# eric-ai-lab/Aerial-Vision-and-Dialog-Navigation

Measured on NVIDIA B200. Metric: HAA-Transformer train episodes/s, higher is better.
Workload: dtype bf16

## Files before the change

### aerial-vision-and-dialog-navigation_b200/_lib.py

```python
from __future__ import annotations

import ctypes as C
import os

import torch

_HERE = os.path.dirname(os.path.abspath(__file__))
LIB_PATH = os.path.join(_HERE, "csrc", "libavdn.so")

_lib = None

c_void_p, c_int, c_i64, c_f32, c_f64 = C.c_void_p, C.c_int, C.c_int64, C.c_float, C.c_double


class ConvItem(C.Structure):
    _fields_ = [("w", C.c_void_p), ("wf", C.c_void_p), ("wd", C.c_void_p), ("dwf", C.c_void_p), ("grad", C.c_void_p),
                ("Cout", C.c_int32), ("Cin", C.c_int32), ("k", C.c_int32), ("stride", C.c_int32),
                ("Cout_p", C.c_int32), ("Cin_p", C.c_int32), ("pairs", C.c_int32), ("pad_", C.c_int32)]


class TileDesc(C.Structure):
    _fields_ = [("tile8", C.c_void_p), ("H", C.c_int32), ("W", C.c_int32)]


_SIGNATURES = {
    "avdn_pack_tile": [c_void_p, c_void_p, c_int, c_int, c_int, c_void_p, c_void_p],
    "avdn_resize_area_width": [c_void_p, c_int, c_int, c_int, c_void_p, c_void_p, c_void_p, c_void_p, c_void_p],
    "avdn_raster_attention": [c_void_p, c_int, c_int, c_void_p, c_int, c_int, c_int, c_void_p, c_void_p],
    "avdn_gps_to_pixels": [c_void_p, c_void_p, c_int, c_void_p, c_void_p],
    "avdn_homography_from_corners": [c_void_p, c_int, c_void_p, c_void_p],
    "avdn_render_views": [c_void_p, c_int, c_void_p, c_void_p, c_int, c_void_p, c_void_p,
                          c_void_p, c_void_p, c_void_p, c_void_p],
    "avdn_gemm_plan": [c_void_p, c_void_p, C.c_size_t],
    "avdn_gemm_run": [c_void_p, c_void_p],
    "avdn_conv0_fwd": [c_void_p, c_void_p, c_void_p, c_int, c_int, c_int, c_void_p, c_void_p],
    "avdn_conv0_fwd_eval": [c_void_p, c_void_p, c_void_p, c_void_p, c_f32, c_void_p, c_int, c_int, c_int, c_void_p],
    "avdn_conv0_wgrad": [c_void_p, c_void_p, c_void_p, c_int, c_int, c_int, c_void_p],
    "avdn_conv0_fwd_stats": [c_void_p, c_void_p, c_int, c_int, c_int, c_void_p, c_void_p, c_void_p, c_void_p],
    "avdn_conv0_fwd_apply": [c_void_p, c_void_p, c_void_p, c_void_p, c_f32, c_void_p, c_void_p, c_int, c_int, c_int,
                             c_void_p],
    "avdn_conv0_set_tensor_path": [c_int],
    "avdn_conv3x3_thin_fwd": [c_void_p, c_void_p, c_void_p, c_int, c_int, c_int, c_int, c_int, c_void_p, c_void_p],
    "avdn_conv3x3_thin_supported": [c_int, c_int, c_int, c_int],
    "avdn_conv3x3_thin_dgrad": [c_void_p, c_void_p, c_void_p, c_int, c_int, c_int, c_int, c_int, c_void_p],
    "avdn_conv3x3_thin_wgrad": [c_void_p, c_void_p, c_void_p, c_int, c_int, c_int, c_int, c_int, c_void_p],
    "avdn_conv0_bwd": [c_void_p] * 8 + [c_f32, c_int, c_int, c_int] + [c_void_p] * 7 + [c_void_p],
    "avdn_bn_stats": [c_void_p, c_i64, c_int, c_int, c_void_p, c_void_p, c_void_p, c_void_p, c_f32, c_f32,
                      c_void_p, c_void_p, c_void_p, c_void_p, c_void_p, c_void_p],
    "avdn_bn_finalize": [c_void_p, c_i64, c_int, c_int, c_void_p, c_void_p, c_void_p, c_void_p, c_f32, c_f32,
                         c_void_p, c_void_p, c_void_p, c_void_p, c_void_p],
    "avdn_bn_eval_coeffs": [c_int, c_int, c_void_p, c_void_p, c_void_p, c_void_p, c_f32, c_void_p, c_void_p,
                            c_void_p],
    "avdn_bn_set_order": [c_int],
    "avdn_bn_apply": [c_void_p, c_void_p, c_void_p, c_void_p, c_void_p, c_i64, c_int, c_f32, c_void_p],
    "avdn_bn_backward": [c_void_p, c_void_p, c_void_p, c_void_p, c_void_p, c_void_p, c_i64, c_int, c_int, c_f32,
                         c_void_p, c_void_p, c_void_p, c_void_p, c_void_p],
    "avdn_bn_backward_apply": [c_void_p, c_void_p, c_void_p, c_void_p, c_void_p, c_void_p, c_i64, c_int, c_int, c_f32,
                               c_void_p, c_void_p, c_void_p, c_void_p, c_void_p, c_void_p],
    "avdn_pack_conv_weight": [c_void_p, c_int, c_int, c_int, c_int, c_int, c_void_p, c_void_p, c_void_p],
    "avdn_unpack_conv_wgrad": [c_void_p, c_int, c_int, c_int, c_int, c_void_p, c_void_p],
    "avdn_unpack_conv_wgrad_pairs": [c_void_p, c_int, c_int, c_int, c_int, c_int, c_int, c_void_p, c_void_p],
    "avdn_pack_conv_weights": [c_void_p, c_int, c_void_p],
    "avdn_unpack_conv_wgrads": [c_void_p, c_int, c_int, c_void_p],
    "avdn_cast_f32_bf16": [c_void_p, c_void_p, c_i64, c_void_p],
    "avdn_nhwc_to_nchw_f32": [c_void_p, c_void_p, c_int, c_int, c_int, c_void_p],
    "avdn_nchw_f32_to_nhwc": [c_void_p, c_void_p, c_int, c_int, c_int, c_void_p],
    "avdn_frame_attn_fwd": [c_void_p] * 6 + [c_int, c_int] + [c_void_p] * 4 + [c_void_p],
    "avdn_frame_attn_bwd": [c_void_p] * 5 + [c_int, c_int] + [c_void_p] * 9 + [c_void_p],
# ... 138 lines not shown
```

### aerial-vision-and-dialog-navigation_b200/csrc/common.cu

```cuda
#include "common.cuh"

#include <stdlib.h>

namespace avdn {

static thread_local char g_err[512] = "ok";

char* err_buf() { return g_err; }

int set_err(int code, const char* fmt, ...) {
  va_list ap;
  va_start(ap, fmt);
  vsnprintf(g_err, sizeof(g_err), fmt, ap);
  va_end(ap);
  return code;
}

int check_launch(const char* what) {
  cudaError_t e = cudaGetLastError();
  if (e != cudaSuccess)
    return set_err(AVDN_ERR_LAUNCH, "%s: %s", what, cudaGetErrorString(e));
  return AVDN_OK;
}

// ... 1 lines not shown
  static int n = 0;
  if (n == 0) {
    int dev = 0;
    if (cudaGetDevice(&dev) != cudaSuccess) return 148;
    cudaDeviceProp p;
    if (cudaGetDeviceProperties(&p, dev) != cudaSuccess) return 148;
    n = p.multiProcessorCount;
  }
  return n;
}

bool pdl_enabled() {
  static const bool on = [] {
    const char* e = getenv("AVDN_PDL");
    return e && e[0] == '1';
  }();
  return on;
}

}

extern "C" const char* avdn_last_error_string(void) { return avdn::err_buf(); }

extern "C" int avdn_abi_version(void) { return 11; }

extern "C" int avdn_device_supported(void) {
  int n = 0;
  if (cudaGetDeviceCount(&n) != cudaSuccess || n == 0) {
    cudaGetLastError();
    return 0;
  }
  cudaDeviceProp p;
  if (cudaGetDeviceProperties(&p, 0) != cudaSuccess) return 0;
  return p.major == 10 ? 1 : 0;
}
```

### aerial-vision-and-dialog-navigation_b200/csrc/conv3_halo.cu

```cuda
#include "common.cuh"
#include "tcgen05.cuh"
#include "conv3_halo.cuh"

namespace {

using namespace avdn_tc;

constexpr int TW = 8, TH = 16;
constexpr int THREADS = 128;

template <int CIN, int COUT, int XBUFS>
struct Cfg {
  static constexpr int ROW = CIN * 2;
  static constexpr int ATOM = 8 * ROW;
  static constexpr int XBOX = (TH + 2) * ATOM;
  static constexpr int XBUF = 3 * XBOX;
  static constexpr int WTAP = COUT * ROW;
  static constexpr int WBYTES = 9 * WTAP;
  static constexpr int OUT_ROW = COUT * 2;
  static constexpr int OUT_BYTES = 128 * OUT_ROW;
  static constexpr int NCH = OUT_ROW / 16;
  static constexpr uint32_t LAYOUT = (CIN == 64) ? 2u : 4u;
  static constexpr int SMEM = XBUFS * XBUF + WBYTES + 2 * OUT_BYTES + 1024;
  static constexpr uint32_t IDESC = (1u << 4) | (1u << 7) | (1u << 10) | ((uint32_t)(COUT >> 3) << 17) | ((uint32_t)(128 >> 4) << 24);
  static constexpr uint32_t TMEM_COLS = COUT < 32 ? 32 : COUT;
// ... 270 lines not shown
    }
  }
  __syncwarp();
  if (n_my > 0) {
    mbar_wait(bar_done, 0);
    tcgen05_fence_after();
    const int co = (int)warp * 16 + (int)lane;
#pragma unroll
    for (int h = 0; h < 9; ++h) {
      uint32_t v[32];
      tmem_ld32(tmem + ((warp * 32u) << 16) + 32 * h, v);
      if (lane < 16) {
        const int kh = h / 3, kw = h % 3;
#pragma unroll
        for (int ci = 0; ci < 32; ++ci) atomicAdd(p.dw + ((co * CIN + ci) * 3 + kh) * 3 + kw, __uint_as_float(v[ci]));
      }
    }
  }
  tcgen05_fence_before();
  __syncthreads();
  if (warp == 0) asm volatile("tcgen05.dealloc.cta_group::1.sync.aligned.b32 %0, %1;" ::"r"(tmem), "r"(512u) : "memory");
}

}

namespace avdn {

static bool tile_ok(int H, int W) { return H % TH == 0 && W % TW == 0 && H >= TH && W >= TW; }

bool conv3_halo_supported(int H, int W, int Cin, int Cout) { return Cin == 32 && Cout == 64 && tile_ok(H, W); }
bool conv3_halo_dgrad_supported(int H, int W, int Cin, int Cout) { return Cin == 32 && Cout == 64 && tile_ok(H, W); }

int conv3_halo_fwd(const void* x, const void* wf, void* z, int N, int H, int W, int Cin, int Cout, double* stats,
                   cudaStream_t s) {
  if (!conv3_halo_supported(H, W, Cin, Cout))
    return set_err(AVDN_ERR_UNSUPPORTED, "conv3_halo: shape %dx%d, %d -> %d channels not covered", H, W, Cin, Cout);
  return stats ? launch<32, 64, false, true, 1>(x, wf, z, N, H, W, stats, s)
               : launch<32, 64, false, false, 1>(x, wf, z, N, H, W, nullptr, s);
}

int conv3_halo_dgrad(const void* dz, const void* wd, void* dx, int N, int H, int W, int Cin, int Cout, cudaStream_t s) {
  if (!conv3_halo_dgrad_supported(H, W, Cin, Cout))
    return set_err(AVDN_ERR_UNSUPPORTED, "conv3_halo dgrad: shape %dx%d, %d -> %d channels not covered", H, W, Cin, Cout);
  return launch<64, 32, true, false, 1>(dz, wd, dx, N, H, W, nullptr, s);
}

int conv3_halo_wgrad(const void* dz, const void* x, float* dw, int N, int H, int W, int Cin, int Cout, cudaStream_t s) {
  if (!conv3_halo_supported(H, W, Cin, Cout))
    return set_err(AVDN_ERR_UNSUPPORTED, "conv3_halo wgrad: shape %dx%d, %d -> %d channels not covered", H, W, Cin, Cout);
  WgParams p;
  const int64_t dx[4] = {Cin, W, H, N}, sx[4] = {1, Cin, (int64_t)W * Cin, (int64_t)H * W * Cin};
  const int32_t bx[4] = {Cin, TW, TH + 2, 1};
  const int64_t dd[4] = {Cout, W, H, N}, sd[4] = {1, Cout, (int64_t)W * Cout, (int64_t)H * W * Cout};
  const int32_t bd[4] = {Cout, TW, TH, 1};
  int r = encode_tensor_map_4d(x, 2, dx, sx, bx, &p.tmX);
  if (!r) r = encode_tensor_map_4d(dz, 2, dd, sd, bd, &p.tmDz);
  if (r) return r;
  p.tiles_x = W / TW;
  p.tiles_y = H / TH;
  const long long nt = (long long)N * p.tiles_x * p.tiles_y;
  if (nt >= (1ll << 31)) return set_err(AVDN_ERR_UNSUPPORTED, "conv3_halo wgrad: too many tiles");
  p.n_tiles = (int32_t)nt;
  p.dw = dw;
  const int smem = WG_STAGES * (3 * (TH + 2) * 8 * 64 + 128 * 128) + 1024;
  static bool attr = false;
  if (!attr) {
    if (cudaFuncSetAttribute(conv3_halo_wgrad_kernel, cudaFuncAttributeMaxDynamicSharedMemorySize, smem) != cudaSuccess)
// ... 8 lines not shown
}

extern "C" int avdn_conv3x3_thin_wgrad(const void* dz, const void* x_nhwc, float* dw, int N, int H, int W, int Cin,
                                       int Cout, avdn_stream_t stream) {
  AVDN_REQUIRE(dz && x_nhwc && dw && N > 0, "avdn_conv3x3_thin_wgrad: bad argument");
  return avdn::conv3_halo_wgrad(dz, x_nhwc, dw, N, H, W, Cin, Cout, avdn::to_cuda(stream));
}

extern "C" int avdn_conv3x3_thin_fwd(const void* x_nhwc, const void* w_f, void* z, int N, int H, int W, int Cin,
                                     int Cout, double* stats, avdn_stream_t stream) {
  AVDN_REQUIRE(x_nhwc && w_f && z && N > 0, "avdn_conv3x3_thin_fwd: bad argument");
  return avdn::conv3_halo_fwd(x_nhwc, w_f, z, N, H, W, Cin, Cout, stats, avdn::to_cuda(stream));
}

extern "C" int avdn_conv3x3_thin_dgrad(const void* dz, const void* w_d, void* dx, int N, int H, int W, int Cin,
                                       int Cout, avdn_stream_t stream) {
  AVDN_REQUIRE(dz && w_d && dx && N > 0, "avdn_conv3x3_thin_dgrad: bad argument");
  return avdn::conv3_halo_dgrad(dz, w_d, dx, N, H, W, Cin, Cout, avdn::to_cuda(stream));
}

extern "C" int avdn_conv3x3_thin_supported(int H, int W, int Cin, int Cout) {
  return avdn::conv3_halo_supported(H, W, Cin, Cout) ? 1 : 0;
}
```

### aerial-vision-and-dialog-navigation_b200/csrc/conv3_halo.cuh

```cuda
#pragma once
#include "common.cuh"

#include <cuda.h>

namespace avdn {

int encode_tensor_map_4d(const void* ptr, int elem_bytes, const int64_t* dim, const int64_t* stride,
                         const int32_t* boxdim, CUtensorMap* out);

bool conv3_halo_supported(int H, int W, int Cin, int Cout);
int conv3_halo_fwd(const void* x, const void* wf, void* z, int N, int H, int W, int Cin, int Cout, double* stats,
                   cudaStream_t s);
bool conv3_halo_dgrad_supported(int H, int W, int Cin, int Cout);
int conv3_halo_dgrad(const void* dz, const void* wd, void* dx, int N, int H, int W, int Cin, int Cout, cudaStream_t s);

int conv3_halo_wgrad(const void* dz, const void* x, float* dw, int N, int H, int W, int Cin, int Cout, cudaStream_t s);

}
```

### aerial-vision-and-dialog-navigation_b200/models/dark_net.py

```python
from __future__ import annotations

import os

import torch
import torch.nn as nn

from .. import _lib
from .. import gemm as G

LEAKY_SLOPE = 0.01
FUSE_BNB = os.environ.get("AVDN_FUSE_BNB", "0") == "1"
CONV0_RECOMPUTE = os.environ.get("AVDN_CONV0_RECOMPUTE", "1") != "0"
CONV_HALO = os.environ.get("AVDN_CONV_HALO", "1") != "0"
BN_EPS = 1e-5
BN_MOMENTUM = 0.1


def parse_model_config(path):
    defs = []
    with open(path, "r") as f:
        for raw in f.read().split("\n"):
            line = raw.strip()
            if not line or line.startswith("#"):
                continue
            if line.startswith("["):
                d = {"type": line[1:-1].rstrip()}
                if d["type"] == "convolutional":
                    d["batch_normalize"] = 0
                defs.append(d)
            else:
                k, v = line.split("=")
                defs[-1][k.rstrip()] = v.strip()
    return defs


def _pad64(c):
# ... 46 lines not shown
        defs = net.module_defs
        out_of = {}
        cur = dict(C=3, Cp=4, H=H, W=W, layer=None)
        shapes = {}
        max_elems = 0
        for i, d in enumerate(defs):
            if d["type"] == "convolutional":
                conv = net.module_list[i][0]
                if int(d["batch_normalize"]) != 1 or d["activation"] != "leaky":
                    raise NotImplementedError("only conv+BN+leaky blocks are on the hot path")
                k, s = conv.kernel_size[0], conv.stride[0]
                if k not in (1, 3) or s not in (1, 2) or (k == 1 and s != 1) or conv.padding[0] != (k - 1) // 2:
                    raise NotImplementedError(f"conv k={k} s={s} pad={conv.padding[0]} is not supported")
                L = _Layer()
                L.idx, L.k, L.s = i, k, s
                L.Cin, L.Cout = conv.in_channels, conv.out_channels
                L.Cin_p = 4 if len(self.layers) == 0 else _pad64(L.Cin)
                L.Cout_p = _pad64(L.Cout)
                L.Hin, L.Win = cur["H"], cur["W"]
                L.Hout, L.Wout = L.Hin // s, L.Win // s
                L.src = cur["layer"]
                L.res = None
                L.first = len(self.layers) == 0
                L.halo = L.halo_dgrad = L.halo_wgrad = False
                if L.first and not (L.Cin == 3 and L.Cout == 32 and k == 3 and s == 1):
                    raise NotImplementedError("first layer must be the 3->32 3x3 stride-1 conv of yolov3")
                L.R = N * L.Hout * L.Wout
                L.flops = 2 * L.R * L.Cout * L.Cin * k * k
                self.layers.append(L)
                out_of[i] = L
                shapes[i] = (L.Cout, L.Hout, L.Wout)
                cur = dict(C=L.Cout, Cp=L.Cout_p, H=L.Hout, W=L.Wout, layer=L)
            elif d["type"] == "shortcut":
                frm = i + int(d["from"]) if int(d["from"]) < 0 else int(d["from"])
                prev = out_of.get(i - 1)
                srcl = out_of.get(frm)
                if prev is None or srcl is None or prev.idx != i - 1 or prev.res is not None:
                    raise NotImplementedError("shortcut must directly follow a convolutional block")
                if shapes[frm] != shapes[i - 1]:
                    raise ValueError("shortcut operands differ in shape")
                prev.res = srcl
                out_of[i] = prev
                shapes[i] = shapes[i - 1]
        self.last = self.layers[-1]
        for L in self.layers:
            n_el = L.R * L.Cout_p
            if not (L.first and CONV0_RECOMPUTE):
# ... 15 lines not shown
                L.wf = torch.empty((L.Cout_p, L.k * L.k * L.Cin_p), dtype=bf, device=dev)
                L.wd = torch.empty((L.Cin_p, L.k * L.k * L.Cout_p), dtype=bf, device=dev)
            L.g = None
        self.x_in = None
        self.dz = None
        self._max_elems = max_elems
        self._fwd_plans = False
        self._eval_plans = False
        self._bwd_plans = False
        self.launches = 0

    def build_fwd(self, x_nhwc4):
        if self._fwd_plans and self.x_in is x_nhwc4:
            return
        self.x_in = x_nhwc4
        if not self._fwd_plans:
            for L in self.layers:
                if L.first:
                    continue
                L.p_fwd = G.plan_conv_fwd(L.src.a, L.wf, L.z, N=self.N, H=L.Hin, W=L.Win, Cin=L.Cin_p,
                                          Cout=L.Cout_p, k=L.k, stride=L.s, flops=L.flops)
                L.p_fwd_stats = G.plan_conv_fwd(L.src.a, L.wf, L.z, N=self.N, H=L.Hin, W=L.Win, Cin=L.Cin_p,
                                                Cout=L.Cout_p, k=L.k, stride=L.s, flops=L.flops, stats=L.sums)
                L.halo = bool(CONV_HALO and L.k == 3 and L.s == 1 and
                              _lib.lib().avdn_conv3x3_thin_supported(L.Hin, L.Win, L.Cin_p, L.Cout_p))
            self._fwd_plans = True

    def conv_table(self, net):
        import ctypes as C
        import numpy as np
        tc = [L for L in self.layers if not L.first]
        sig = tuple((net.module_list[L.idx][0].weight.data_ptr(),
                     0 if getattr(L, "dwf", None) is None else L.dwf.data_ptr(),
                     0 if getattr(L, "dw", None) is None else L.dw.data_ptr()) for L in tc)
        if getattr(self, "_table_sig", None) != sig:
            arr = (_lib.ConvItem * len(tc))()
            for i, L in enumerate(tc):
                it = arr[i]
                it.w = net.module_list[L.idx][0].weight.data_ptr()
                it.wf, it.wd = L.wf.data_ptr(), L.wd.data_ptr()
                it.dwf, it.grad = sig[i][1] or None, sig[i][2] or None
                if getattr(L, "halo_wgrad", False):
                    it.dwf = None
                it.Cout, it.Cin, it.k, it.stride = L.Cout, L.Cin, L.k, L.s
                it.Cout_p, it.Cin_p = L.Cout_p, L.Cin_p
                it.pairs = 1 if getattr(L, "pairs", False) else 0
            raw = np.frombuffer(bytes(arr), dtype=np.uint8).copy()
            self._table = torch.from_numpy(raw).to(self.device)
# ... 103 lines not shown
    for li, L in enumerate(eng.layers):
        conv = net.module_list[L.idx][0]
        bn = net.module_list[L.idx][1]
        if not train:
            if not reuse:
                call("avdn_bn_eval_coeffs", L.Cout_p, L.Cout, ptr(bn.weight), ptr(bn.bias), ptr(bn.running_mean),
                     ptr(bn.running_var), BN_EPS, ptr(L.scale), ptr(L.shift))
                n += 1
            if L.first:
                call("avdn_conv0_fwd_eval", ptr(x_nhwc4), ptr(conv.weight), ptr(L.scale), ptr(L.shift), LEAKY_SLOPE,
                     ptr(L.a), eng.N, L.Hin, L.Win)
                n += 1
            else:
                L.p_fwd_eval.run()
                n += 1
            continue
        if L.first and L.recompute:
            call("avdn_conv0_fwd_stats", ptr(x_nhwc4), ptr(conv.weight), eng.N, L.Hin, L.Win, ptr(L.sums), ptr(L.zw),
                 ptr(L.xs9))
            n += 2
        elif L.first:
            call("avdn_conv0_fwd", ptr(x_nhwc4), ptr(conv.weight), ptr(L.z), eng.N, L.Hin, L.Win, ptr(L.sums))
            n += 1
        elif L.halo:
            call("avdn_conv3x3_thin_fwd", ptr(L.src.a), ptr(L.wf), ptr(L.z), eng.N, L.Hin, L.Win, L.Cin_p, L.Cout_p,
                 ptr(L.sums), flops=L.flops)
            n += 1
        else:
            L.p_fwd_stats.run()
            n += 1
        call("avdn_bn_finalize", ptr(L.sums), L.R, L.Cout_p, L.Cout, ptr(bn.weight), ptr(bn.bias),
             ptr(bn.running_mean), ptr(bn.running_var), BN_MOMENTUM, BN_EPS, ptr(L.scale),
             ptr(L.shift), ptr(L.mean), ptr(L.rstd))
        n += 1
        if L.first and L.recompute:
            call("avdn_conv0_fwd_apply", ptr(x_nhwc4), ptr(conv.weight), ptr(L.scale), ptr(L.shift), LEAKY_SLOPE,
                 ptr(L.a), ptr(L.mask), eng.N, L.Hin, L.Win)
        else:
            call("avdn_bn_apply", ptr(L.z), ptr(L.scale), ptr(L.shift), ptr(L.res.a) if L.res is not None else None,
                 ptr(L.a), L.R, L.Cout_p, LEAKY_SLOPE)
        n += 1
    if train:
        net._bump_batches_tracked()
    last = eng.last
    if out is None:
        out = torch.empty((eng.N, last.Cout, last.Hout, last.Wout), dtype=torch.float32, device=eng.device)
    call("avdn_nhwc_to_nchw_f32", ptr(last.a), ptr(out), eng.N, last.Hout * last.Wout, last.Cout_p)
    eng.launches += n + 1
# ... 21 lines not shown


def _layer_backward(eng, L, unpack=True, zero=True):
    call, ptr = _lib.call, _lib.ptr
    if L.first and L.recompute:
        conv = eng.net_ref().module_list[L.idx][0]
        call("avdn_conv0_bwd", ptr(eng.x_in), ptr(conv.weight), ptr(L.g), ptr(L.mask), ptr(L.scale), ptr(L.shift), ptr(L.mean),
             ptr(L.rstd), LEAKY_SLOPE, eng.N, L.Hin, L.Win, ptr(L.zw), ptr(L.xs9), ptr(L.sums), ptr(L.gw), ptr(L.dw),
             ptr(L.dgamma), ptr(L.dbeta))
        return 2
    if L.bnb_fused and L.bnb_ready:
        call("avdn_bn_backward_apply", ptr(L.g), ptr(L.z), ptr(L.scale), ptr(L.shift), ptr(L.mean), ptr(L.rstd), L.R,
             L.Cout_p, L.Cout, LEAKY_SLOPE, ptr(L.bsums), ptr(L.coef), ptr(L.dz), ptr(L.dgamma), ptr(L.dbeta))
        L.bnb_ready = False
        n = 2
    else:
        call("avdn_bn_backward", ptr(L.g), ptr(L.z), ptr(L.scale), ptr(L.shift), ptr(L.mean), ptr(L.rstd), L.R,
             L.Cout_p, L.Cout, LEAKY_SLOPE, ptr(L.sums), ptr(L.dz), ptr(L.dgamma), ptr(L.dbeta))
        n = 3
    if L.first:
        call("avdn_conv0_wgrad", ptr(L.dz), ptr(eng.x_in), ptr(L.dw), eng.N, L.Hin, L.Win)
        return n + 1
    if L.halo_wgrad:
        call("avdn_conv3x3_thin_wgrad", ptr(L.dz), ptr(L.src.a), ptr(L.dw), eng.N, L.Hin, L.Win, L.Cin_p, L.Cout_p,
             flops=L.flops)
        n += 1
        unpack = False
    else:
        if zero:
            L.dwf.zero_()
            n += 1
        L.p_wgrad.run()
        n += 1
    if unpack:
        if L.pairs:
            call("avdn_unpack_conv_wgrad_pairs", ptr(L.dwf), L.Cout, L.Cin, L.k, L.s, L.Cout_p, L.Cin_p, ptr(L.dw))
        else:
            call("avdn_unpack_conv_wgrad", ptr(L.dwf), L.Cout, L.Cin, L.k, L.Cin_p, ptr(L.dw))
        n += 1
    if L.src.bnb_fused:
        if zero:
            L.src.bsums.zero_()
            n += 1
        L.src.bnb_ready = True
    if L.halo_dgrad:
        call("avdn_conv3x3_thin_dgrad", ptr(L.dz), ptr(L.wd), ptr(L.src.g), eng.N, L.Hin, L.Win, L.Cin_p,
             L.Cout_p, flops=L.flops)
        return n + 1
    for p in L.p_dgrad:
        p.run()
    return n + len(L.p_dgrad)


def _trunk_backward(net, eng, dout, after_layer=None, flush_layers=None):
    call, ptr = _lib.call, _lib.ptr
    eng.build_bwd(net)
    tbl = eng.conv_table(net)
    last = eng.last
    eng.dwf_arena.zero_()
    n = 2
    call("avdn_nchw_f32_to_nhwc", ptr(dout), ptr(last.g), eng.N, last.Hout * last.Wout, last.Cout_p)
    flush = set(flush_layers or ())
    hi = len(eng.layers) - 1
    for li in reversed(range(len(eng.layers))):
        n += _layer_backward(eng, eng.layers[li], unpack=False, zero=False)
        if li in flush or li == 0:
            lo = max(li, 1)
            if hi >= lo:
                call("avdn_unpack_conv_wgrads", ptr(tbl), lo - 1, hi - lo + 1)
# ... 90 lines not shown
```

### include/avdn.h

```cpp
#ifndef AVDN_H_
#define AVDN_H_

#include <stddef.h>
#include <stdint.h>

#ifdef __cplusplus
extern "C" {
#endif

typedef struct CUstream_st* avdn_stream_t;

typedef enum avdn_status {
  AVDN_OK = 0,
  AVDN_ERR_BAD_ARG = -1,
  AVDN_ERR_UNSUPPORTED = -2,
  AVDN_ERR_LAUNCH = -3,
  AVDN_ERR_NO_DEVICE = -4,
  AVDN_ERR_DRIVER = -5
} avdn_status;

const char* avdn_last_error_string(void);
int avdn_abi_version(void);
int avdn_device_supported(void);

// ... 97 lines not shown
int avdn_conv0_fwd(const void* x_nhwc4, const float* w, void* z, int N, int H, int W, double* stats,
                   avdn_stream_t stream);
int avdn_conv0_fwd_eval(const void* x_nhwc4, const float* w, const float* scale, const float* shift, float slope,
                        void* a, int N, int H, int W, avdn_stream_t stream);
int avdn_conv0_wgrad(const void* dz, const void* x_nhwc4, float* dw, int N, int H, int W, avdn_stream_t stream);
int avdn_conv0_set_tensor_path(int on);
int avdn_conv0_fwd_stats(const void* x_nhwc4, const float* w, int N, int H, int W, double* stats, float* zw,
                         double* xs9, avdn_stream_t stream);
int avdn_conv0_fwd_apply(const void* x_nhwc4, const float* w, const float* scale, const float* shift, float slope,
                         void* a, void* mask, int N, int H, int W, avdn_stream_t stream);
int avdn_conv0_bwd(const void* x_nhwc4, const float* w, const void* da, const void* mask, const float* scale,
                   const float* shift,
                   const float* mean, const float* rstd, float slope, int N, int H, int W, const float* zw,
                   const double* xs9, double* sums, float* gw, float* dw, float* dgamma, float* dbeta,
                   avdn_stream_t stream);

int avdn_conv3x3_thin_fwd(const void* x_nhwc, const void* w_f, void* z, int N, int H, int W, int Cin, int Cout,
                          double* stats, avdn_stream_t stream);
int avdn_conv3x3_thin_supported(int H, int W, int Cin, int Cout);
int avdn_conv3x3_thin_dgrad(const void* dz, const void* w_d, void* dx, int N, int H, int W, int Cin, int Cout,
                            avdn_stream_t stream);
int avdn_conv3x3_thin_wgrad(const void* dz, const void* x_nhwc, float* dw, int N, int H, int W, int Cin, int Cout,
                            avdn_stream_t stream);

int avdn_bn_stats(const void* z, long long R, int C, int C_real, const float* gamma, const float* beta,
                  float* running_mean, float* running_var, float momentum, float eps, double* sums,
                  float* scale, float* shift, float* mean, float* rstd, avdn_stream_t stream);
int avdn_bn_finalize(const double* sums, long long R, int C, int C_real, const float* gamma, const float* beta,
                     float* running_mean, float* running_var, float momentum, float eps, float* scale,
                     float* shift, float* mean, float* rstd, avdn_stream_t stream);
int avdn_bn_eval_coeffs(int C, int C_real, const float* gamma, const float* beta, const float* running_mean,
                        const float* running_var, float eps, float* scale, float* shift, avdn_stream_t stream);
int avdn_bn_apply(const void* z, const float* scale, const float* shift, const void* residual, void* a,
                  long long R, int C, float slope, avdn_stream_t stream);
int avdn_bn_backward(const void* da, const void* z, const float* scale, const float* shift, const float* mean,
                     const float* rstd, long long R, int C, int C_real, float slope, double* sums, void* dz,
                     float* dgamma, float* dbeta, avdn_stream_t stream);
int avdn_bn_backward_apply(const void* da, const void* z, const float* scale, const float* shift,
                           const float* mean, const float* rstd, long long R, int C, int C_real, float slope,
                           const double* sums, float* coef, void* dz, float* dgamma, float* dbeta,
                           avdn_stream_t stream);

int avdn_bn_set_order(int mask);

int avdn_pack_conv_weight(const float* w, int Cout, int Cin, int k, int Cout_p, int Cin_p, void* wf, void* wd,
                          avdn_stream_t stream);
// ... 149 lines not shown
```

Measured before the change: 1133.

## Add halo-tiled tcgen05 stride-2 3x3 conv dgrad and wgrad kernels

Adds dedicated stride-2 3x3 conv kernels (forward, dgrad, wgrad) for the 32->64 channel layer, using TMA loads of even/odd pixel-pair views, tcgen05 MMAs into tensor memory and warp-specialized pipelines. The layer table now enables the halo path for stride-2 layers in backward (dgrad/wgrad), while the stride-2 forward stays on the generic path because halo_fwd is restricted to stride 1. This targets the implicit-GEMM/im2col overhead of the generic path for this layer. It adds substantial new kernel code, with correctness risks around pair-view descriptors and atomics in wgrad.

```diff
diff --git a/aerial-vision-and-dialog-navigation_b200/_lib.py b/aerial-vision-and-dialog-navigation_b200/_lib.py
--- a/aerial-vision-and-dialog-navigation_b200/_lib.py
+++ b/aerial-vision-and-dialog-navigation_b200/_lib.py
@@ -44,6 +44,10 @@
     "avdn_conv3x3_thin_supported": [c_int, c_int, c_int, c_int],
     "avdn_conv3x3_thin_dgrad": [c_void_p, c_void_p, c_void_p, c_int, c_int, c_int, c_int, c_int, c_void_p],
     "avdn_conv3x3_thin_wgrad": [c_void_p, c_void_p, c_void_p, c_int, c_int, c_int, c_int, c_int, c_void_p],
+    "avdn_conv3x3_thin_s2_fwd": [c_void_p, c_void_p, c_void_p, c_int, c_int, c_int, c_int, c_int, c_void_p, c_void_p],
+    "avdn_conv3x3_thin_s2_supported": [c_int, c_int, c_int, c_int],
+    "avdn_conv3x3_thin_s2_dgrad": [c_void_p, c_void_p, c_void_p, c_int, c_int, c_int, c_int, c_int, c_void_p],
+    "avdn_conv3x3_thin_s2_wgrad": [c_void_p, c_void_p, c_void_p, c_int, c_int, c_int, c_int, c_int, c_void_p],
     "avdn_conv0_bwd": [c_void_p] * 8 + [c_f32, c_int, c_int, c_int] + [c_void_p] * 7 + [c_void_p],
     "avdn_bn_stats": [c_void_p, c_i64, c_int, c_int, c_void_p, c_void_p, c_void_p, c_void_p, c_f32, c_f32,
                       c_void_p, c_void_p, c_void_p, c_void_p, c_void_p, c_void_p],
diff --git a/aerial-vision-and-dialog-navigation_b200/csrc/common.cu b/aerial-vision-and-dialog-navigation_b200/csrc/common.cu
--- a/aerial-vision-and-dialog-navigation_b200/csrc/common.cu
+++ b/aerial-vision-and-dialog-navigation_b200/csrc/common.cu
@@ -47,7 +47,7 @@
 
 extern "C" const char* avdn_last_error_string(void) { return avdn::err_buf(); }
 
-extern "C" int avdn_abi_version(void) { return 11; }
+extern "C" int avdn_abi_version(void) { return 12; }
 
 extern "C" int avdn_device_supported(void) {
   int n = 0;
diff --git a/aerial-vision-and-dialog-navigation_b200/csrc/conv3_halo.cu b/aerial-vision-and-dialog-navigation_b200/csrc/conv3_halo.cu
--- a/aerial-vision-and-dialog-navigation_b200/csrc/conv3_halo.cu
+++ b/aerial-vision-and-dialog-navigation_b200/csrc/conv3_halo.cu
@@ -1,6 +1,8 @@
 #include "common.cuh"
 #include "tcgen05.cuh"
 #include "conv3_halo.cuh"
+
+#include <type_traits>
 
 namespace {
 
@@ -317,6 +319,330 @@
   if (warp == 0) asm volatile("tcgen05.dealloc.cta_group::1.sync.aligned.b32 %0, %1;" ::"r"(tmem), "r"(512u) : "memory");
 }
 
+struct S2Fwd {
+  static constexpr int STAGES = 2, STAGE = 2 * 17 * 1024 + 2 * 16 * 1024;
+  static constexpr int WBYTES = 6 * 8192;
+  static constexpr int TILE_KINDS = 1;
+};
+struct S2Dgrad {
+  static constexpr int STAGES = 4, STAGE = 2 * 17 * 1024;
+  static constexpr int WBYTES = 9 * 4096;
+  static constexpr int TILE_KINDS = 2;
+};
+constexpr int S2_THREADS = 192;
+constexpr uint32_t S2_IDESC_N64 = (1u << 4) | (1u << 7) | (1u << 10) | ((uint32_t)(64 >> 3) << 17) | ((uint32_t)(128 >> 4) << 24);
+constexpr uint32_t S2_IDESC_N32 = (1u << 4) | (1u << 7) | (1u << 10) | ((uint32_t)(32 >> 3) << 17) | ((uint32_t)(128 >> 4) << 24);
+constexpr int S2_OUT_BYTES = 128 * 128;
+
+template <class V>
+constexpr int s2_smem() { return V::STAGES * V::STAGE + V::WBYTES + 2 * S2_OUT_BYTES + 1024; }
+
+struct alignas(64) S2Params {
+  CUtensorMap tmA[2];
+  CUtensorMap tmW;
+  CUtensorMap tmO[2];
+  int32_t tiles_x, tiles_y, n_tiles;
+  double* stats;
+};
+
+template <bool DGRAD, bool STATS>
+__global__ void __launch_bounds__(S2_THREADS, 1) conv3_s2_kernel(const __grid_constant__ S2Params p) {
+  using V = std::conditional_t<DGRAD, S2Dgrad, S2Fwd>;
+  constexpr int S = V::STAGES, ATOM = 1024;
+  extern __shared__ uint8_t smem_raw[];
+  const uint32_t base = (smem_u32(smem_raw) + 1023u) & ~1023u;
+  const uint32_t ws = base + S * V::STAGE, outs = ws + V::WBYTES;
+  __shared__ __align__(8) uint64_t bars[2 * S + 5];
+  __shared__ uint32_t tmem_slot;
+  const uint32_t bar_full = smem_u32(&bars[0]), bar_empty = bar_full + 8 * S, bar_w = bar_empty + 8 * S,
+                 bar_accf = bar_w + 8, bar_acce = bar_accf + 16;
+  const uint32_t tid = threadIdx.x, warp = tid >> 5, lane = tid & 31;
+  if (tid == 0) {
+    for (int s = 0; s < S; ++s) { mbar_init(bar_full + 8 * s, 1); mbar_init(bar_empty + 8 * s, 1); }
+    mbar_init(bar_w, 1);
+    for (int a = 0; a < 2; ++a) { mbar_init(bar_accf + 8 * a, 1); mbar_init(bar_acce + 8 * a, 4); }
+    asm volatile("fence.mbarrier_init.release.cluster;" ::: "memory");
+  }
+  if (warp == 1) {
+    asm volatile("tcgen05.alloc.cta_group::1.sync.aligned.shared::cta.b32 [%0], %1;" ::"r"(smem_u32(&tmem_slot)), "r"(128u)
+                 : "memory");
+    asm volatile("tcgen05.relinquish_alloc_permit.cta_group::1.sync.aligned;" ::: "memory");
+  }
+  tcgen05_fence_before();
+  __syncthreads();
+  tcgen05_fence_after();
+  const uint32_t tmem = tmem_slot;
+  const int per_img = V::TILE_KINDS * p.tiles_x * p.tiles_y;
+  const int n_my = ((int)blockIdx.x < p.n_tiles) ? (p.n_tiles - 1 - (int)blockIdx.x) / (int)gridDim.x + 1 : 0;
+  auto decode = [&](int tile, int& n, int& kind, int& ty, int& tx) {
+    n = tile / per_img;
+    int r = tile - n * per_img;
+    kind = r % V::TILE_KINDS;
+    r /= V::TILE_KINDS;
+    ty = r / p.tiles_x;
+    tx = r - ty * p.tiles_x;
+  };
+
+  if (warp == 0) {
+    if (elect_one() && n_my > 0) {
+      if (DGRAD) {
+        mbar_expect_tx(bar_w, (uint32_t)V::WBYTES);
+        for (int t = 0; t < 9; ++t) tma_load_4d<1>(ws + t * 4096, &p.tmW, bar_w, t * 64, 0, 0, 0);
+      } else {
+        mbar_expect_tx(bar_w, (uint32_t)V::WBYTES);
+        for (int kh = 0; kh < 3; ++kh) {
+          tma_load_4d<1>(ws + (2 * kh) * 8192, &p.tmW, bar_w, (3 * kh - 1) * 32, 0, 0, 0);
+          tma_load_4d<1>(ws + (2 * kh + 1) * 8192, &p.tmW, bar_w, (3 * kh + 1) * 32, 0, 0, 0);
+        }
+      }
+      for (int it = 0; it < n_my; ++it) {
+        const int s = it % S, use = it / S;
+        if (use > 0) mbar_wait(bar_empty + 8 * s, (uint32_t)(use - 1) & 1u);
+        int n, kind, ty, tx;
+        decode((int)blockIdx.x + it * (int)gridDim.x, n, kind, ty, tx);
+        const uint32_t sx = base + s * V::STAGE, fb = bar_full + 8 * s;
+        mbar_expect_tx(fb, (uint32_t)V::STAGE);
+        if (DGRAD) {
+          tma_load_4d<1>(sx, &p.tmA[0], fb, 0, tx * TW, ty * TH, n);
+          tma_load_4d<1>(sx + 17 * ATOM, &p.tmA[0], fb, 0, tx * TW + 1, ty * TH, n);
+        } else {
+          tma_load_4d<1>(sx, &p.tmA[0], fb, 0, tx * TW - 1, ty * TH - 1, n);
+          tma_load_4d<1>(sx + 17 * ATOM, &p.tmA[0], fb, 0, tx * TW, ty * TH - 1, n);
+          tma_load_4d<1>(sx + 34 * ATOM, &p.tmA[1], fb, 0, tx * TW - 1, ty * TH, n);
+          tma_load_4d<1>(sx + 50 * ATOM, &p.tmA[1], fb, 0, tx * TW, ty * TH, n);
+        }
+      }
+    }
+  } else if (warp == 1) {
+    if (elect_one() && n_my > 0) {
+      mbar_wait(bar_w, 0);
+      for (int it = 0; it < n_my; ++it) {
+        const int s = it % S, a = it & 1;
+        mbar_wait(bar_full + 8 * s, (uint32_t)(it / S) & 1u);
+        if (it >= 2) mbar_wait(bar_acce + 8 * a, (uint32_t)((it >> 1) - 1) & 1u);
+        tcgen05_fence_after();
+        const uint32_t sx = base + s * V::STAGE, d = tmem + 64u * (uint32_t)a;
+        if (DGRAD) {
+          int n, kind, ty, tx;
+          decode((int)blockIdx.x + it * (int)gridDim.x, n, kind, ty, tx);
+          for (int j = 0; j < 1 + kind; ++j) {
+            const int kh = kind ? 2 * j : 1, off = (kind && j == 0) ? 1 : 0;
+            const uint64_t a0 = make_smem_desc(sx + off * ATOM, 16, 1024, 2);
+            const uint64_t a1 = make_smem_desc(sx + (17 + off) * ATOM, 16, 1024, 2);
+            const uint64_t b0 = make_smem_desc(ws + (3 * kh) * 4096, 16, 1024, 2);
+            const uint64_t b1 = make_smem_desc(ws + (3 * kh + 1) * 4096, 16, 1024, 2);
+            const uint64_t b2 = make_smem_desc(ws + (3 * kh + 2) * 4096, 16, 1024, 2);
+#pragma unroll
+            for (int k = 0; k < 4; ++k)
+              umma_bf16<1>(d, a0 + (uint64_t)(2 * k), b1 + (uint64_t)(2 * k), S2_IDESC_N32, (j > 0 || k > 0) ? 1u : 0u);
+#pragma unroll
+            for (int k = 0; k < 4; ++k)
+              umma_bf16<1>(d + 32, a1 + (uint64_t)(2 * k), b0 + (uint64_t)(2 * k), S2_IDESC_N32, (j > 0 || k > 0) ? 1u : 0u);
+#pragma unroll
+            for (int k = 0; k < 4; ++k) umma_bf16<1>(d + 32, a0 + (uint64_t)(2 * k), b2 + (uint64_t)(2 * k), S2_IDESC_N32, 1u);
+          }
+        } else {
+          uint32_t acc = 0u;
+#pragma unroll
+          for (int kh = 0; kh < 3; ++kh) {
+            const uint32_t view = (kh == 1) ? sx + 34 * ATOM : sx, box = (kh == 1) ? 16 * ATOM : 17 * ATOM;
+            const uint32_t off = (kh == 2) ? ATOM : 0u;
+            const uint64_t am = make_smem_desc(view + off, 16, 1024, 2), a0 = make_smem_desc(view + box + off, 16, 1024, 2);
+            const uint64_t bm = make_smem_desc(ws + (2 * kh) * 8192, 16, 1024, 2);
+            const uint64_t b0 = make_smem_desc(ws + (2 * kh + 1) * 8192, 16, 1024, 2);
+#pragma unroll
+            for (int k = 2; k < 4; ++k) {
+              umma_bf16<1>(d, am + (uint64_t)(2 * k), bm + (uint64_t)(2 * k), S2_IDESC_N64, acc);
+              acc = 1u;
+            }
+#pragma unroll
+            for (int k = 0; k < 4; ++k) umma_bf16<1>(d, a0 + (uint64_t)(2 * k), b0 + (uint64_t)(2 * k), S2_IDESC_N64, 1u);
+          }
+        }
+        tcgen05_commit<1>(bar_empty + 8 * s);
+        tcgen05_commit<1>(bar_accf + 8 * a);
+      }
+    }
+  } else {
+    const uint32_t e = tid - 64, m = 32u * (warp & 3u) + lane;
+    float s1[8], s2[8];
+#pragma unroll
+    for (int j = 0; j < 8; ++j) s1[j] = s2[j] = 0.f;
+    for (int it = 0; it < n_my; ++it) {
+      const int a = it & 1;
+      mbar_wait(bar_accf + 8 * a, (uint32_t)(it >> 1) & 1u);
+      tcgen05_fence_after();
+      const uint32_t slab = outs + (uint32_t)a * S2_OUT_BYTES;
+#pragma unroll
+      for (int h = 0; h < 2; ++h) {
+        uint32_t v[32];
+        tmem_ld32(tmem + ((32u * (warp & 3u)) << 16) + 64u * (uint32_t)a + 32 * h, v);
+#pragma unroll
+        for (int c = 0; c < 4; ++c)
+          sts128(slab + out_chunk<128>(m, (uint32_t)(4 * h + c)),
+                 pack2(__uint_as_float(v[8 * c]), __uint_as_float(v[8 * c + 1])),
+                 pack2(__uint_as_float(v[8 * c + 2]), __uint_as_float(v[8 * c + 3])),
+                 pack2(__uint_as_float(v[8 * c + 4]), __uint_as_float(v[8 * c + 5])),
+                 pack2(__uint_as_float(v[8 * c + 6]), __uint_as_float(v[8 * c + 7])));
+      }
+      tcgen05_fence_before();
+      __syncwarp();
+      if (lane == 0) mbar_arrive(bar_acce + 8 * a);
+      fence_proxy_async_smem();
+      asm volatile("bar.sync 1, 128;" ::: "memory");
+      if (e == 0) {
+        int n, kind, ty, tx;
+        decode((int)blockIdx.x + it * (int)gridDim.x, n, kind, ty, tx);
+        tma_store_4d(&p.tmO[DGRAD ? kind : 0], slab, 0, tx * TW, ty * TH, n);
+        tma_commit_group();
+      }
+      if (STATS) {
+        const uint32_t cj = e % 8;
+#pragma unroll
+        for (int i = 0; i < 8; ++i) {
+          const uint4 v = lds128(slab + out_chunk<128>(e / 8 + 16u * i, cj));
+          const uint32_t w4[4] = {v.x, v.y, v.z, v.w};
+#pragma unroll
+          for (int k = 0; k < 4; ++k) {
+            const float lo = __uint_as_float(w4[k] << 16), hi = __uint_as_float(w4[k] & 0xFFFF0000u);
+            s1[2 * k] += lo; s2[2 * k] = fmaf(lo, lo, s2[2 * k]);
+            s1[2 * k + 1] += hi; s2[2 * k + 1] = fmaf(hi, hi, s2[2 * k + 1]);
+          }
+        }
+      }
+      if (e == 0) tma_wait_group_read<1>();
+      asm volatile("bar.sync 1, 128;" ::: "memory");
+    }
+    if (e == 0) tma_wait_group_read<0>();
+    asm volatile("bar.sync 1, 128;" ::: "memory");
+    if (STATS && p.stats != nullptr && n_my > 0) {
+      float* s_red = reinterpret_cast<float*>(smem_raw + (outs - smem_u32(smem_raw)));
+      const int j = (int)e % 8, g = (int)e / 8;
+#pragma unroll
+      for (int k = 0; k < 8; ++k) { s_red[g * 64 + j * 8 + k] = s1[k]; s_red[(16 + g) * 64 + j * 8 + k] = s2[k]; }
+      asm volatile("bar.sync 1, 128;" ::: "memory");
+      const int which = (int)e / 64, c = (int)e % 64;
+      float acc = 0.f;
+      for (int g2 = 0; g2 < 16; ++g2) acc += s_red[(which * 16 + g2) * 64 + c];
+      atomicAdd(p.stats + which * 64 + c, (double)acc);
+    }
+    if (e == 0) asm volatile("cp.async.bulk.wait_group 0;" ::: "memory");
+  }
+  tcgen05_fence_before();
+  __syncthreads();
+  if (warp == 1) asm volatile("tcgen05.dealloc.cta_group::1.sync.aligned.b32 %0, %1;" ::"r"(tmem), "r"(128u) : "memory");
+}
+
+constexpr int S2W_STAGES = 2, S2W_XBUF = 66 * 1024, S2W_STAGE = S2W_XBUF + 128 * 128;
+struct alignas(64) S2WgParams {
+  CUtensorMap tmXo, tmXe, tmDz;
+  int32_t tiles_x, tiles_y, n_tiles;
+  float* dw;
+};
+
+__global__ void __launch_bounds__(THREADS, 1) conv3_s2_wgrad_kernel(const __grid_constant__ S2WgParams p) {
+  constexpr int CIN = 32, ATOM = 1024;
+  extern __shared__ uint8_t smem_raw[];
+  const uint32_t base = (smem_u32(smem_raw) + 1023u) & ~1023u;
+  __shared__ __align__(8) uint64_t bars[2 * S2W_STAGES + 1];
+  __shared__ uint32_t tmem_slot;
+  const uint32_t bar_full = smem_u32(&bars[0]), bar_free = bar_full + 8 * S2W_STAGES, bar_done = bar_free + 8 * S2W_STAGES;
+  const uint32_t tid = threadIdx.x, warp = tid >> 5, lane = tid & 31;
+  if (tid == 0) {
+    for (int s = 0; s < S2W_STAGES; ++s) { mbar_init(bar_full + 8 * s, 1); mbar_init(bar_free + 8 * s, 1); }
+    mbar_init(bar_done, 1);
+    asm volatile("fence.mbarrier_init.release.cluster;" ::: "memory");
+  }
+  if (warp == 0) {
+    asm volatile("tcgen05.alloc.cta_group::1.sync.aligned.shared::cta.b32 [%0], %1;" ::"r"(smem_u32(&tmem_slot)), "r"(512u)
+                 : "memory");
+    asm volatile("tcgen05.relinquish_alloc_permit.cta_group::1.sync.aligned;" ::: "memory");
+  }
+  tcgen05_fence_before();
+  __syncthreads();
+  tcgen05_fence_after();
+  const uint32_t tmem = tmem_slot;
+  const int per_img = p.tiles_x * p.tiles_y;
+  const int n_my = ((int)blockIdx.x < p.n_tiles) ? (p.n_tiles - 1 - (int)blockIdx.x) / (int)gridDim.x + 1 : 0;
+
+  if (tid == 0) {
+    for (int it = 0; it < n_my; ++it) {
+      const int s = it % S2W_STAGES, use = it / S2W_STAGES;
+      if (use > 0) mbar_wait(bar_free + 8 * s, (uint32_t)(use - 1) & 1u);
+      const int tile = (int)blockIdx.x + it * (int)gridDim.x;
+      const int n = tile / per_img, r = tile - n * per_img, ty = r / p.tiles_x, tx = r - ty * p.tiles_x;
+      const uint32_t sx = base + s * S2W_STAGE, fb = bar_full + 8 * s;
+      mbar_expect_tx(fb, (uint32_t)S2W_STAGE);
+      tma_load_4d<1>(sx, &p.tmXo, fb, 0, tx * TW - 1, ty * TH - 1, n);
+      tma_load_4d<1>(sx + 17 * ATOM, &p.tmXo, fb, 0, tx * TW, ty * TH - 1, n);
+      tma_load_4d<1>(sx + 34 * ATOM, &p.tmXe, fb, 0, tx * TW - 1, ty * TH, n);
+      tma_load_4d<1>(sx + 50 * ATOM, &p.tmXe, fb, 0, tx * TW, ty * TH, n);
+      tma_load_4d<1>(sx + S2W_XBUF, &p.tmDz, fb, 0, tx * TW, ty * TH, n);
+    }
+  } else if (tid == 32) {
+    constexpr uint32_t IDESC = (1u << 4) | (1u << 7) | (1u << 10) | (1u << 15) | (1u << 16) | ((uint32_t)(128 >> 3) << 17) |
+                               ((uint32_t)(64 >> 4) << 24);
+    for (int it = 0; it < n_my; ++it) {
+      const int s = it % S2W_STAGES, use = it / S2W_STAGES;
+      mbar_wait(bar_full + 8 * s, (uint32_t)use & 1u);
+      tcgen05_fence_after();
+      const uint32_t sx = base + s * S2W_STAGE;
+      const uint64_t ad = make_smem_desc(sx + S2W_XBUF, 16384, 1024, 2);
+#pragma unroll
+      for (int kh = 0; kh < 3; ++kh) {
+        const uint64_t bd = (kh == 1) ? make_smem_desc(sx + 34 * ATOM, 16 * ATOM, 1024, 2)
+                                      : make_smem_desc(sx + (kh == 2 ? ATOM : 0), 17 * ATOM, 1024, 2);
+#pragma unroll
+        for (int k = 0; k < 8; ++k)
+          umma_bf16<1>(tmem + 128 * kh, ad + (uint64_t)(k * 128), bd + (uint64_t)(k * 128), IDESC, (it > 0 || k > 0) ? 1u : 0u);
+      }
+      tcgen05_commit<1>(bar_free + 8 * s);
+      if (it == n_my - 1) tcgen05_commit<1>(bar_done);
+    }
+  }
+  __syncwarp();
+  if (n_my > 0) {
+    mbar_wait(bar_done, 0);
+    tcgen05_fence_after();
+    const int co = (int)warp * 16 + (int)lane;
+#pragma unroll
+    for (int h = 0; h < 12; ++h) {
+      if (h % 4 == 0) continue;
+      uint32_t v[32];
+      tmem_ld32(tmem + ((warp * 32u) << 16) + 32 * h, v);
+      if (lane < 16) {
+        const int kh = h / 4, kw = h % 4 - 1;
+#pragma unroll
+        for (int ci = 0; ci < 32; ++ci) atomicAdd(p.dw + ((co * CIN + ci) * 3 + kh) * 3 + kw, __uint_as_float(v[ci]));
+      }
+    }
+  }
+  tcgen05_fence_before();
+  __syncthreads();
+  if (warp == 0) asm volatile("tcgen05.dealloc.cta_group::1.sync.aligned.b32 %0, %1;" ::"r"(tmem), "r"(512u) : "memory");
+}
+
+int encode_pair_view(const void* t, int N, int H, int W, int py, int rows, CUtensorMap* out) {
+  const int64_t d[4] = {64, W / 2, H / 2, N}, st[4] = {1, 64, 2ll * W * 32, (int64_t)H * W * 32};
+  const int32_t b[4] = {64, TW, rows, 1};
+  return avdn::encode_tensor_map_4d(static_cast<const __nv_bfloat16*>(t) + (int64_t)py * W * 32, 2, d, st, b, out);
+}
+
+template <bool DGRAD, bool STATS>
+int launch_s2(const S2Params& p, cudaStream_t s) {
+  using V = std::conditional_t<DGRAD, S2Dgrad, S2Fwd>;
+  auto kfn = conv3_s2_kernel<DGRAD, STATS>;
+  static bool attr = false;
+  if (!attr) {
+    if (cudaFuncSetAttribute(kfn, cudaFuncAttributeMaxDynamicSharedMemorySize, s2_smem<V>()) != cudaSuccess)
+      return avdn::check_launch("conv3_s2 smem attribute");
+    attr = true;
+  }
+  const long long cap = avdn::sm_count();
+  kfn<<<(unsigned)(p.n_tiles < cap ? p.n_tiles : cap), S2_THREADS, s2_smem<V>(), s>>>(p);
+  return avdn::check_launch("conv3_s2_kernel");
+}
+
 }
 
 namespace avdn {
@@ -338,6 +664,90 @@
   if (!conv3_halo_dgrad_supported(H, W, Cin, Cout))
     return set_err(AVDN_ERR_UNSUPPORTED, "conv3_halo dgrad: shape %dx%d, %d -> %d channels not covered", H, W, Cin, Cout);
   return launch<64, 32, true, false, 1>(dz, wd, dx, N, H, W, nullptr, s);
+}
+
+bool conv3_halo_s2_supported(int H, int W, int Cin, int Cout) {
+  return Cin == 32 && Cout == 64 && H % (2 * TH) == 0 && W % (2 * TW) == 0 && H >= 2 * TH && W >= 2 * TW;
+}
+
+static int s2_tiles(int N, int H, int W, int kinds, S2Params& p, const char* what) {
+  p.tiles_x = W / 2 / TW;
+  p.tiles_y = H / 2 / TH;
+  const long long nt = (long long)N * kinds * p.tiles_x * p.tiles_y;
+  if (nt >= (1ll << 31)) return set_err(AVDN_ERR_UNSUPPORTED, "%s: too many tiles", what);
+  p.n_tiles = (int32_t)nt;
+  return AVDN_OK;
+}
+
+int conv3_halo_s2_fwd(const void* x, const void* wf, void* z, int N, int H, int W, int Cin, int Cout, double* stats,
+                      cudaStream_t s) {
+  if (!conv3_halo_s2_supported(H, W, Cin, Cout))
+    return set_err(AVDN_ERR_UNSUPPORTED, "conv3_halo s2: shape %dx%d, %d -> %d channels not covered", H, W, Cin, Cout);
+  S2Params p;
+  const int64_t dw[4] = {9 * 32, 64, 1, 1}, sw[4] = {1, 9 * 32, 9 * 32 * 64, 9 * 32 * 64};
+  const int32_t bw[4] = {64, 64, 1, 1};
+  const int64_t dz[4] = {64, W / 2, H / 2, N}, sz[4] = {1, 64, (int64_t)W / 2 * 64, (int64_t)H / 2 * W / 2 * 64};
+  const int32_t bz[4] = {64, TW, TH, 1};
+  int r = encode_pair_view(x, N, H, W, 1, TH + 1, &p.tmA[0]);
+  if (!r) r = encode_pair_view(x, N, H, W, 0, TH, &p.tmA[1]);
+  if (!r) r = encode_tensor_map_4d(wf, 2, dw, sw, bw, &p.tmW);
+  if (!r) r = encode_tensor_map_4d(z, 2, dz, sz, bz, &p.tmO[0]);
+  if (!r) p.tmO[1] = p.tmO[0];
+  if (!r) r = s2_tiles(N, H, W, 1, p, "conv3_halo s2");
+  if (r) return r;
+  p.stats = stats;
+  if (stats && cudaMemsetAsync(stats, 0, sizeof(double) * 2 * 64, s) != cudaSuccess)
+    return check_launch("conv3_halo s2 stats memset");
+  return stats ? launch_s2<false, true>(p, s) : launch_s2<false, false>(p, s);
+}
+
+int conv3_halo_s2_dgrad(const void* dz, const void* wd, void* dx, int N, int H, int W, int Cin, int Cout, cudaStream_t s) {
+  if (!conv3_halo_s2_supported(H, W, Cin, Cout))
+    return set_err(AVDN_ERR_UNSUPPORTED, "conv3_halo s2 dgrad: shape %dx%d, %d -> %d channels not covered", H, W, Cin,
+                   Cout);
+  S2Params p;
+  const int64_t dd[4] = {64, W / 2, H / 2, N}, sd[4] = {1, 64, (int64_t)W / 2 * 64, (int64_t)H / 2 * W / 2 * 64};
+  const int32_t bd[4] = {64, TW, TH + 1, 1};
+  const int64_t dw[4] = {9 * 64, 32, 1, 1}, sw[4] = {1, 9 * 64, 9 * 64 * 32, 9 * 64 * 32};
+  const int32_t bw[4] = {64, 32, 1, 1};
+  int r = encode_tensor_map_4d(dz, 2, dd, sd, bd, &p.tmA[0]);
+  if (!r) p.tmA[1] = p.tmA[0];
+  if (!r) r = encode_tensor_map_4d(wd, 2, dw, sw, bw, &p.tmW);
+  if (!r) r = encode_pair_view(dx, N, H, W, 0, TH, &p.tmO[0]);
+  if (!r) r = encode_pair_view(dx, N, H, W, 1, TH, &p.tmO[1]);
+  if (!r) r = s2_tiles(N, H, W, 2, p, "conv3_halo s2 dgrad");
+  if (r) return r;
+  p.stats = nullptr;
+  return launch_s2<true, false>(p, s);
+}
+
+int conv3_halo_s2_wgrad(const void* dz, const void* x, float* dw, int N, int H, int W, int Cin, int Cout, cudaStream_t s) {
+  if (!conv3_halo_s2_supported(H, W, Cin, Cout))
+    return set_err(AVDN_ERR_UNSUPPORTED, "conv3_halo s2 wgrad: shape %dx%d, %d -> %d channels not covered", H, W, Cin,
+                   Cout);
+  S2WgParams p;
+  const int64_t dd[4] = {64, W / 2, H / 2, N}, sd[4] = {1, 64, (int64_t)W / 2 * 64, (int64_t)H / 2 * W / 2 * 64};
+  const int32_t bd[4] = {64, TW, TH, 1};
+  int r = encode_pair_view(x, N, H, W, 1, TH + 1, &p.tmXo);
+  if (!r) r = encode_pair_view(x, N, H, W, 0, TH, &p.tmXe);
+  if (!r) r = encode_tensor_map_4d(dz, 2, dd, sd, bd, &p.tmDz);
+  if (r) return r;
+  p.tiles_x = W / 2 / TW;
+  p.tiles_y = H / 2 / TH;
+  const long long nt = (long long)N * p.tiles_x * p.tiles_y;
+  if (nt >= (1ll << 31)) return set_err(AVDN_ERR_UNSUPPORTED, "conv3_halo s2 wgrad: too many tiles");
+  p.n_tiles = (int32_t)nt;
+  p.dw = dw;
+  constexpr int smem = S2W_STAGES * S2W_STAGE + 1024;
+  static bool attr = false;
+  if (!attr) {
+    if (cudaFuncSetAttribute(conv3_s2_wgrad_kernel, cudaFuncAttributeMaxDynamicSharedMemorySize, smem) != cudaSuccess)
+      return check_launch("conv3_halo s2 wgrad smem attribute");
+    attr = true;
+  }
+  const long long cap = sm_count();
+  conv3_s2_wgrad_kernel<<<(unsigned)(nt < cap ? nt : cap), THREADS, smem, s>>>(p);
+  return check_launch("conv3_s2_wgrad_kernel");
 }
 
 int conv3_halo_wgrad(const void* dz, const void* x, float* dw, int N, int H, int W, int Cin, int Cout, cudaStream_t s) {
@@ -392,3 +802,25 @@
 extern "C" int avdn_conv3x3_thin_supported(int H, int W, int Cin, int Cout) {
   return avdn::conv3_halo_supported(H, W, Cin, Cout) ? 1 : 0;
 }
+
+extern "C" int avdn_conv3x3_thin_s2_supported(int H, int W, int Cin, int Cout) {
+  return avdn::conv3_halo_s2_supported(H, W, Cin, Cout) ? 1 : 0;
+}
+
+extern "C" int avdn_conv3x3_thin_s2_fwd(const void* x_nhwc, const void* w_f, void* z, int N, int H, int W, int Cin,
+                                        int Cout, double* stats, avdn_stream_t stream) {
+  AVDN_REQUIRE(x_nhwc && w_f && z && N > 0, "avdn_conv3x3_thin_s2_fwd: bad argument");
+  return avdn::conv3_halo_s2_fwd(x_nhwc, w_f, z, N, H, W, Cin, Cout, stats, avdn::to_cuda(stream));
+}
+
+extern "C" int avdn_conv3x3_thin_s2_dgrad(const void* dz, const void* w_d, void* dx, int N, int H, int W, int Cin,
+                                          int Cout, avdn_stream_t stream) {
+  AVDN_REQUIRE(dz && w_d && dx && N > 0, "avdn_conv3x3_thin_s2_dgrad: bad argument");
+  return avdn::conv3_halo_s2_dgrad(dz, w_d, dx, N, H, W, Cin, Cout, avdn::to_cuda(stream));
+}
+
+extern "C" int avdn_conv3x3_thin_s2_wgrad(const void* dz, const void* x_nhwc, float* dw, int N, int H, int W, int Cin,
+                                          int Cout, avdn_stream_t stream) {
+  AVDN_REQUIRE(dz && x_nhwc && dw && N > 0, "avdn_conv3x3_thin_s2_wgrad: bad argument");
+  return avdn::conv3_halo_s2_wgrad(dz, x_nhwc, dw, N, H, W, Cin, Cout, avdn::to_cuda(stream));
+}
diff --git a/aerial-vision-and-dialog-navigation_b200/csrc/conv3_halo.cuh b/aerial-vision-and-dialog-navigation_b200/csrc/conv3_halo.cuh
--- a/aerial-vision-and-dialog-navigation_b200/csrc/conv3_halo.cuh
+++ b/aerial-vision-and-dialog-navigation_b200/csrc/conv3_halo.cuh
@@ -16,4 +16,10 @@
 
 int conv3_halo_wgrad(const void* dz, const void* x, float* dw, int N, int H, int W, int Cin, int Cout, cudaStream_t s);
 
+bool conv3_halo_s2_supported(int H, int W, int Cin, int Cout);
+int conv3_halo_s2_fwd(const void* x, const void* wf, void* z, int N, int H, int W, int Cin, int Cout, double* stats,
+                      cudaStream_t s);
+int conv3_halo_s2_dgrad(const void* dz, const void* wd, void* dx, int N, int H, int W, int Cin, int Cout, cudaStream_t s);
+int conv3_halo_s2_wgrad(const void* dz, const void* x, float* dw, int N, int H, int W, int Cin, int Cout, cudaStream_t s);
+
 }
diff --git a/aerial-vision-and-dialog-navigation_b200/models/dark_net.py b/aerial-vision-and-dialog-navigation_b200/models/dark_net.py
--- a/aerial-vision-and-dialog-navigation_b200/models/dark_net.py
+++ b/aerial-vision-and-dialog-navigation_b200/models/dark_net.py
@@ -12,6 +12,7 @@
 FUSE_BNB = os.environ.get("AVDN_FUSE_BNB", "0") == "1"
 CONV0_RECOMPUTE = os.environ.get("AVDN_CONV0_RECOMPUTE", "1") != "0"
 CONV_HALO = os.environ.get("AVDN_CONV_HALO", "1") != "0"
+_THIN = {1: "avdn_conv3x3_thin_", 2: "avdn_conv3x3_thin_s2_"}
 BN_EPS = 1e-5
 BN_MOMENTUM = 0.1
 
@@ -104,7 +105,7 @@
                 L.src = cur["layer"]
                 L.res = None
                 L.first = len(self.layers) == 0
-                L.halo = L.halo_dgrad = L.halo_wgrad = False
+                L.halo = L.halo_fwd = L.halo_dgrad = L.halo_wgrad = False
                 if L.first and not (L.Cin == 3 and L.Cout == 32 and k == 3 and s == 1):
                     raise NotImplementedError("first layer must be the 3->32 3x3 stride-1 conv of yolov3")
                 L.R = N * L.Hout * L.Wout
@@ -166,8 +167,9 @@
                                           Cout=L.Cout_p, k=L.k, stride=L.s, flops=L.flops)
                 L.p_fwd_stats = G.plan_conv_fwd(L.src.a, L.wf, L.z, N=self.N, H=L.Hin, W=L.Win, Cin=L.Cin_p,
                                                 Cout=L.Cout_p, k=L.k, stride=L.s, flops=L.flops, stats=L.sums)
-                L.halo = bool(CONV_HALO and L.k == 3 and L.s == 1 and
-                              _lib.lib().avdn_conv3x3_thin_supported(L.Hin, L.Win, L.Cin_p, L.Cout_p))
+                L.halo = bool(CONV_HALO and L.k == 3 and
+                              getattr(_lib.lib(), _THIN[L.s] + "supported")(L.Hin, L.Win, L.Cin_p, L.Cout_p))
+                L.halo_fwd = L.halo and L.s == 1
             self._fwd_plans = True
 
     def conv_table(self, net):
@@ -317,8 +319,8 @@
         elif L.first:
             call("avdn_conv0_fwd", ptr(x_nhwc4), ptr(conv.weight), ptr(L.z), eng.N, L.Hin, L.Win, ptr(L.sums))
             n += 1
-        elif L.halo:
-            call("avdn_conv3x3_thin_fwd", ptr(L.src.a), ptr(L.wf), ptr(L.z), eng.N, L.Hin, L.Win, L.Cin_p, L.Cout_p,
+        elif L.halo_fwd:
+            call(_THIN[L.s] + "fwd", ptr(L.src.a), ptr(L.wf), ptr(L.z), eng.N, L.Hin, L.Win, L.Cin_p, L.Cout_p,
                  ptr(L.sums), flops=L.flops)
             n += 1
         else:
@@ -386,7 +388,7 @@
         call("avdn_conv0_wgrad", ptr(L.dz), ptr(eng.x_in), ptr(L.dw), eng.N, L.Hin, L.Win)
         return n + 1
     if L.halo_wgrad:
-        call("avdn_conv3x3_thin_wgrad", ptr(L.dz), ptr(L.src.a), ptr(L.dw), eng.N, L.Hin, L.Win, L.Cin_p, L.Cout_p,
+        call(_THIN[L.s] + "wgrad", ptr(L.dz), ptr(L.src.a), ptr(L.dw), eng.N, L.Hin, L.Win, L.Cin_p, L.Cout_p,
              flops=L.flops)
         n += 1
         unpack = False
@@ -408,7 +410,7 @@
             n += 1
         L.src.bnb_ready = True
     if L.halo_dgrad:
-        call("avdn_conv3x3_thin_dgrad", ptr(L.dz), ptr(L.wd), ptr(L.src.g), eng.N, L.Hin, L.Win, L.Cin_p,
+        call(_THIN[L.s] + "dgrad", ptr(L.dz), ptr(L.wd), ptr(L.src.g), eng.N, L.Hin, L.Win, L.Cin_p,
              L.Cout_p, flops=L.flops)
         return n + 1
     for p in L.p_dgrad:
diff --git a/include/avdn.h b/include/avdn.h
--- a/include/avdn.h
+++ b/include/avdn.h
@@ -143,6 +143,13 @@
                             avdn_stream_t stream);
 int avdn_conv3x3_thin_wgrad(const void* dz, const void* x_nhwc, float* dw, int N, int H, int W, int Cin, int Cout,
                             avdn_stream_t stream);
+int avdn_conv3x3_thin_s2_fwd(const void* x_nhwc, const void* w_f, void* z, int N, int H, int W, int Cin, int Cout,
+                             double* stats, avdn_stream_t stream);
+int avdn_conv3x3_thin_s2_supported(int H, int W, int Cin, int Cout);
+int avdn_conv3x3_thin_s2_dgrad(const void* dz, const void* w_d, void* dx, int N, int H, int W, int Cin, int Cout,
+                               avdn_stream_t stream);
+int avdn_conv3x3_thin_s2_wgrad(const void* dz, const void* x_nhwc, float* dw, int N, int H, int W, int Cin, int Cout,
+                               avdn_stream_t stream);
 
 int avdn_bn_stats(const void* z, long long R, int C, int C_real, const float* gamma, const float* beta,
                   float* running_mean, float* running_var, float momentum, float eps, double* sums,
```

New measurement: 1158 (median of 6 runs). 1.02x the previous value.
